# szcompressor/SZ3

Hardware: AMD Instinct MI355X
Metric: compression throughput GB/s + ratio at fixed abs errBound, 512^3 f32 (higher is better)
Workload: dtype f32; 1 GPU; C2: 3D float32 512x512x512 synthetic field per GPU, Lorenzo predictor, abs errBound=0.001, device-resident in -> device-resident Huffman payload; parallelism=slab1, algo=HIP_LORENZO(16), exchange=none (one rank)

## Files before the change

### include/sz3hip.h

```cpp
#ifndef SZ3HIP_H
#define SZ3HIP_H
#include <stddef.h>
#include <stdint.h>
#include "sz3hip_debug.h"

#ifdef __cplusplus
extern "C" {
#endif

#define SZ3HIP_FLOAT 0
#define SZ3HIP_DOUBLE 1
#define SZ3HIP_UINT8 2
#define SZ3HIP_INT8 3
#define SZ3HIP_UINT16 4
#define SZ3HIP_INT16 5
#define SZ3HIP_UINT32 6
#define SZ3HIP_INT32 7
#define SZ3HIP_UINT64 8
#define SZ3HIP_INT64 9

enum { SZ3HIP_EB_ABS = 0, SZ3HIP_EB_REL, SZ3HIP_EB_PSNR, SZ3HIP_EB_L2NORM, SZ3HIP_EB_ABS_AND_REL, SZ3HIP_EB_ABS_OR_REL };

enum {
    SZ3HIP_ALGO_LORENZO_REG = 0,
// ... 136 lines not shown
void sz3hip_set_profiling(sz3hip_ctx *ctx, int on);
int sz3hip_get_stage_times(sz3hip_ctx *ctx, const char **names, float *ms, int max);
void sz3hip_ctx_forget(sz3hip_ctx *ctx);
void sz3hip_ctx_set_speculation(sz3hip_ctx *ctx, int off);
void sz3hip_ctx_set_deterministic(sz3hip_ctx *ctx, int on);
void sz3hip_ctx_set_tuner_exact(sz3hip_ctx *ctx, int on);
void sz3hip_get_spec_stats(const sz3hip_ctx *ctx, uint32_t *hits, uint32_t *misses);
int sz3hip_last_call_fused(const sz3hip_ctx *ctx);
int sz3hip_last_call_q16(const sz3hip_ctx *ctx);
void sz3hip_ctx_set_fused(sz3hip_ctx *ctx, int on);
int sz3hip_lab_build(void);
int sz3hip_debug_copy_codes(sz3hip_ctx *ctx, uint16_t *host_codes, uint64_t n);
int sz3hip_debug_decode_info(sz3hip_ctx *ctx, uint32_t *out4);
void sz3hip_debug_force_generic(int on);
void sz3hip_debug_flags(int flags);

typedef struct sz3hip_comm sz3hip_comm;
#define SZ3HIP_COMM_ID_BYTES 128
sz3hip_comm *sz3hip_comm_create_local(int ndev, const int *devices);
int sz3hip_comm_unique_id(unsigned char *id128);
sz3hip_comm *sz3hip_comm_create_rank(int nranks, int rank, int device, const unsigned char *id128);
void sz3hip_comm_destroy(sz3hip_comm *comm);
int sz3hip_comm_size(const sz3hip_comm *comm);
int sz3hip_comm_rank(const sz3hip_comm *comm);
int sz3hip_comm_local_size(const sz3hip_comm *comm);
int sz3hip_comm_device(const sz3hip_comm *comm, int member);
int sz3hip_comm_allreduce_histogram(sz3hip_comm *comm, sz3hip_ctx *const *ctxs, void *const *streams);
int sz3hip_comm_allreduce_u64(sz3hip_comm *comm, void *const *d_bufs, size_t count, void *const *streams);
int sz3hip_comm_allreduce_minmax(sz3hip_comm *comm, double *mins, double *maxs, void *const *streams);

// ... 11 lines not shown
```

### include/sz3hip_debug.h

```cpp
#ifndef SZ3HIP_DEBUG_H
#define SZ3HIP_DEBUG_H

enum sz3hip_dbg {
    SZ3HIP_DBG_CB_COMPACT_IN_WG = 1,
    SZ3HIP_DBG_K1_LAB_NO_HIST = 1,
    SZ3HIP_DBG_DEC_MULTI_SYM = 2,
    SZ3HIP_DBG_K1_NO_CODE_STORES = 2,
    SZ3HIP_DBG_BLKDEC_FORCE_RETRY = 4,
    SZ3HIP_DBG_K1_V4_NO_STENCIL = 4,
    SZ3HIP_DBG_K1_NO_Q16 = 8,
    SZ3HIP_DBG_BLKDEC_LOCAL_EXPANDED = 16,
    SZ3HIP_DBG_K1_V4_NO_PREFETCH = 16,
    SZ3HIP_DBG_PACK_LAB_NO_STORES = 16,
    SZ3HIP_DBG_K1_NO_MARCH = 32,
    SZ3HIP_DBG_K1_NO_NARROW = 64,
    SZ3HIP_DBG_INTERP_NO_VEC = 128,
    SZ3HIP_DBG_K1_NO_WIDTH_SPEC = 256,
    SZ3HIP_DBG_DEC_NO_FUSED_X = 512,
    SZ3HIP_DBG_PACK_LAB_ONE_UNIT = 512,
    SZ3HIP_DBG_CB_ONE_CLASS = 1024,
    SZ3HIP_DBG_K1_NO_FUSED = 2048,
    SZ3HIP_DBG_BLK_RANK_3_LAUNCHES = 2048,
    SZ3HIP_DBG_BLK_SIDE_8_LAUNCHES = 2048,
    SZ3HIP_DBG_K1_NO_XCD_ORDER = 4096,
// ... 12 lines not shown
    SZ3HIP_DBG_INTERP_LEVELS_ANY_SIZE = 4194304,
    SZ3HIP_DBG_K1_NO_SAMP_IN_LAUNCH = 4194304,
    SZ3HIP_DBG_BLKDEC_BLOCK_PER_WAVE = 8388608,
    SZ3HIP_DBG_K1_Q16_PLAIN_STORES = 8388608,
    SZ3HIP_DBG_K1_NO_DEFER_FOLD = 16777216,
    SZ3HIP_DBG_PACK_NO_SEG_BITS = 33554432,
    SZ3HIP_DBG_BLK_FIT_TILES = 67108864,
    SZ3HIP_DBG_BLK_1D_WAVE_PER_BLOCK = 134217728,
    SZ3HIP_DBG_CTX_NO_PUBLISH_ZERO = 268435456,
    SZ3HIP_DBG_INTERP_HANDOVER_IN_PLACE = 536870912,
    SZ3HIP_DBG_DEC_CARRY_PASS = 536870912,
    SZ3HIP_DBG_BLK_NO_EXIT = 1073741824,
    SZ3HIP_DBG_BLK_NO_SELECT = -2147483647 - 1
};

#endif
```

### sz3_amd/__init__.py

```python
import contextlib
import ctypes as C
import enum
import os

import numpy as np

_HERE = os.path.dirname(os.path.abspath(__file__))
LIB_PATH = os.environ.get("SZ3HIP_LIB") or os.path.join(_HERE, "libsz3hip.so")

EB_ABS, EB_REL, EB_PSNR, EB_L2NORM, EB_ABS_AND_REL, EB_ABS_OR_REL = range(6)
ALGO_LORENZO_REG, ALGO_INTERP_LORENZO, ALGO_INTERP, ALGO_NOPRED, ALGO_LOSSLESS = range(5)
ALGO_HIP_LORENZO = 16
ALGO_HIP_INTERP = 17
INTERP_ALGO_LINEAR, INTERP_ALGO_CUBIC = 0, 1
SZ_FLOAT, SZ_DOUBLE = 0, 1


class Dbg(enum.IntFlag):
    CB_COMPACT_IN_WG = 1
    K1_LAB_NO_HIST = 1
    DEC_MULTI_SYM = 2
    K1_NO_CODE_STORES = 2
    BLKDEC_FORCE_RETRY = 4
    K1_V4_NO_STENCIL = 4
# ... 25 lines not shown
    DEC_DIRECT_STORES = 1048576
    DEC_NO_HALF = 2097152
    INTERP_LEVELS_ANY_SIZE = 4194304
    K1_NO_SAMP_IN_LAUNCH = 4194304
    BLKDEC_BLOCK_PER_WAVE = 8388608
    K1_Q16_PLAIN_STORES = 8388608
    K1_NO_DEFER_FOLD = 16777216
    PACK_NO_SEG_BITS = 33554432
    BLK_FIT_TILES = 67108864
    BLK_1D_WAVE_PER_BLOCK = 134217728
    CTX_NO_PUBLISH_ZERO = 268435456
    INTERP_HANDOVER_IN_PLACE = 536870912
    DEC_CARRY_PASS = 536870912
    BLK_NO_EXIT = 1073741824
    BLK_NO_SELECT = 2147483648


class SZ3HipError(RuntimeError):
    def __init__(self, code, msg):
        super().__init__("sz3hip error %d: %s" % (code, msg))
        self.code = code


class _CConfig(C.Structure):
    _fields_ = [
        ("N", C.c_int32), ("dims", C.c_uint64 * 4), ("num", C.c_uint64),
        ("cmprAlgo", C.c_uint8), ("errorBoundMode", C.c_uint8),
        ("absErrorBound", C.c_double), ("relErrorBound", C.c_double),
        ("psnrErrorBound", C.c_double), ("l2normErrorBound", C.c_double),
        ("openmp", C.c_uint8), ("quantbinCnt", C.c_int32), ("blockSize", C.c_int32),
# ... 234 lines not shown
def _check(rc):
    if rc != 0:
        raise SZ3HipError(rc, lib().sz3hip_last_error().decode())


@contextlib.contextmanager
def debug_flags(flags):
    L = lib()
    L.sz3hip_debug_flags(int(flags))
    try:
        yield
    finally:
        L.sz3hip_debug_flags(0)


_SZ_TYPES = {"float32": 0, "float64": 1, "uint8": 2, "int8": 3, "uint16": 4, "int16": 5, "uint32": 6, "int32": 7, "uint64": 8, "int64": 9}


def _dtype_id(dt):
    dt = np.dtype(dt)
    if dt.name in _SZ_TYPES:
        return _SZ_TYPES[dt.name]
    raise TypeError("sz3_amd supports float32 / float64 and 8 ... 64-bit integers (got %s)" % dt)


class Config:

    _FIELDS = [f[0] for f in _CConfig._fields_ if f[0] not in ("dims",)]

    def __init__(self, *dims):
# ... 544 lines not shown
```

### sz3_amd/csrc/sz3hip_api.cpp

```cpp
#include <hip/hip_runtime.h>

#include <dlfcn.h>
#include <math.h>
#include <stdarg.h>
#include <stdio.h>
#include <stdlib.h>
#include <string.h>

#include <sched.h>
#include <unistd.h>
#include <algorithm>
#include <atomic>
#include <chrono>
#include <mutex>
#include <string>
#include <thread>
#include <vector>

#include "../../include/sz3c.h"
#include "../../include/sz3hip.h"
#include "sz3hip_format.h"
#include "sz3hip_internal.h"
#include "sz3hip_stock_geom.h"
#include "sz3hip_kernels.h"
// ... 1594 lines not shown
        cb.skip_sort = 1;
        int rcb = szk_launch_codebook(ctx->d_hist, &cb, ctx->book_stream);
        if (rcb) return fail(SZ3HIP_EHIP, "codebook kernel launch failed (%d)", rcb);
        HIPCHK(hipEventRecord(ctx->ev_book, ctx->book_stream));
        er.roles = 1;
        er.no_book = 1;
        er.hist = ctx->d_hist;
        er.cb = &cb;
        er.used_lens = ctx->bk[used].lens;
        er.flags = reinterpret_cast<uint32_t *>(ctx->d_counters + 10);
        er.exact = ctx->spec_exact;
    }
    if (how == S2_SAMPLED) {
        er.roles = 1;
        er.no_book = 1;
        er.hist = ctx->d_hist;
        er.cb = &cb;
        er.used_lens = ctx->bk[used].lens;
        er.flags = reinterpret_cast<uint32_t *>(ctx->d_counters + 10);
        er.exact = 1;
    }
    if (how == S2_CLASSIC) {
        if (ctx->range_ready && !cb.range_ready)
            HIPCHK(hipMemsetAsync(ctx->d_counters + 8, 0, 16, s));
        prof_begin(ctx, ST_CODEBOOK, s);
        int rcb = szk_launch_codebook(ctx->d_hist, &cb, s);
        prof_end(ctx, ST_CODEBOOK, s);
        if (rcb) return fail(SZ3HIP_EHIP, "codebook kernel launch failed (%d)", rcb);
    }
    szk_layout_params lp;
// ... 573 lines not shown
    return 1;
#else
    return 0;
#endif
}
extern "C" void sz3hip_ctx_set_fused(sz3hip_ctx *ctx, int on) { ctx->fuse_on = on != 0 && sz3hip_lab_build(); }
extern "C" void sz3hip_get_spec_stats(const sz3hip_ctx *ctx, uint32_t *hits, uint32_t *misses) {
    *hits = ctx->spec_hits;
    *misses = ctx->spec_misses;
}
extern "C" void sz3hip_debug_flags(int flags) {
    szk_dbg_flags = flags;
    szk_interp_novec = (flags & SZ3HIP_DBG_INTERP_NO_VEC) != 0;
    szk_interp_min_blocks = (flags & SZ3HIP_DBG_INTERP_LEVELS_ANY_SIZE) ? 1 : 256;
}
extern "C" int sz3hip_debug_codebook_info(sz3hip_ctx *ctx, uint64_t *out16) {
    HIPCHK(hipSetDevice(ctx->device));
    HIPCHK(hipDeviceSynchronize());
    szk_cb_info info;
    HIPCHK(hipMemcpy(&info, ctx->bk[ctx->book_idx < 0 ? 0 : ctx->book_idx].info, sizeof(info), hipMemcpyDeviceToHost));
    out16[0] = info.n_symbols; out16[1] = info.max_len; out16[2] = info.sym_min; out16[3] = info.sym_count;
    for (int i = 0; i < 12; i++) out16[4 + i] = info.ts[i];
    return 0;
}

extern "C" int sz3hip_debug_decode_info(sz3hip_ctx *ctx, uint32_t *out4) {
    out4[0] = ctx->last_half;
    out4[1] = ctx->last_carry;
    out4[2] = (uint32_t)ctx->half_skip;
    out4[3] = 0;
// ... 287 lines not shown
```

### sz3_amd/csrc/sz3hip_kernels.h

```cpp
#ifndef SZ3HIP_KERNELS_H
#define SZ3HIP_KERNELS_H
#include <hip/hip_runtime.h>
#include <stdint.h>
#include "sz3hip_format.h"
#include "../../include/sz3hip_debug.h"

struct szk_lattice {
    double recip, two_eb, eb;
    float recip_f, two_eb_f, eb_lo_f;
};
static inline szk_lattice szk_make_lattice(double eb) {
    szk_lattice l;
    l.eb = eb;
    l.two_eb = 2.0 * eb;
    l.recip = 1.0 / l.two_eb;
    l.recip_f = (float)l.recip;
    l.two_eb_f = (float)l.two_eb;
    float e = (float)eb;
    if ((double)e > eb) e = __builtin_nextafterf(e, 0.0f);
    l.eb_lo_f = e;
    return l;
}

#define SZK_K1_GRID 2048u
// ... 137 lines not shown
    const uint8_t *side;
    int lists_by_roles;
    int assumed_narrow;
    const uint32_t *q16_flag;
    szk_mode mode;
    const uint32_t *samp_words;
};
struct szk_merge_args {
    const uint32_t *slots;
    const uint32_t *seg_base;
    const uint32_t *fuse_flag;
};
struct szk_encode_roles {
    int roles;
    int no_book;
    const uint64_t *hist;
    const szk_cb_params *cb;
    const uint8_t *used_lens;
    uint32_t *flags;
    int exact;
    const uint32_t *fold_partial;
    uint32_t fold_rows;
    uint64_t *fold_hist;
    uint32_t *fold_range;
};
#define SZK_PACKB_ONLY_SAMPLED 1u
#define SZK_PACKB_LAB_NO_STORES 8u
#define SZK_PACKB_LAB_ONE_UNIT 16u

#define DEC_LUT_BITS 12u
// ... 271 lines not shown
                          uint32_t radius ,
                          uint32_t esc_sym ,
                          uint32_t *zero_word ,
                          const uint16_t *chunk_words, uint64_t n_chunks, uint64_t *group_off, uint64_t *total_words , hipStream_t s);
int szk_launch_decode(const uint8_t *payload, const szk_dec_params *p, uint16_t *codes, uint64_t *chunk_off,
                      uint64_t *total_words, hipStream_t s);
int szk_launch_reconstruct(int x_done, const uint8_t *payload, const szh_header *h, const szh_offsets *o, const uint16_t *codes,
                           void *d_out, void *d_segtot, hipStream_t s, const uint32_t *gate = nullptr,
                           const void *carry = nullptr );
int szk_half_scans_ok(const szh_header *h);
int szk_launch_reconstruct_half(const uint8_t *payload, const szh_header *h, const szh_offsets *o, void *d_half ,
                                void *d_out, uint32_t *ovf, hipStream_t s, const void *carry = nullptr );
void szk_host_offsets(const szh_header *h, szh_offsets *o);
extern int szk_force_generic;
extern int szk_dbg_flags;

#endif
```

### sz3_amd/csrc/sz3hip_kernels.hip

```cpp
#include <hip/hip_runtime.h>
#include <cstddef>
#include <stdint.h>
#include <type_traits>
#include <mutex>
#include <utility>
#include <vector>
#include "sz3hip_format.h"
#include "sz3hip_kernels.h"

#include "sz3hip_devutil.h"

template <typename T>
__global__ __launch_bounds__(256) void k_minmax(const T *__restrict__ in, uint64_t n, double *partial) {
    double mn = INFINITY, mx = -INFINITY;
    bool has_nan = false;
    for (uint64_t i = (uint64_t)blockIdx.x * blockDim.x + threadIdx.x; i < n; i += (uint64_t)gridDim.x * blockDim.x) {
        double v = (double)in[i];
        if (v < mn) mn = v;
        if (v > mx) mx = v;
        has_nan |= (v != v);
    }
    (void)has_nan;
#pragma unroll
    for (int d = WAVE / 2; d > 0; d >>= 1) {
// ... 3498 lines not shown
            tot += s_w[w];
        }
#pragma unroll
        for (int j = 0; j < SCAN_GPT; j++) {
            if (gt + j < n_groups) group_off[gt + j] = run;
            run += sum[j];
        }
        __syncthreads();
        if (threadIdx.x == 0) s_carry += tot;
        __syncthreads();
    }
    if (threadIdx.x == 0) *total_words = s_carry;
}
__global__ __launch_bounds__(256) void k_seg_chunks(const uint16_t *__restrict__ seg_bits, uint64_t n_segs, const uint32_t *seg_made,
                                                    uint16_t *__restrict__ chunk_words, uint64_t n_chunks, uint32_t *__restrict__ group_sums,
                                                    uint16_t *__restrict__ sub_bits) {
    const bool seg_ok = *seg_made != 0;
    const uint64_t n_vec = (n_segs + 7) / 8;
    const uint64_t n_vec16 = (n_vec + 15) / 16 * 16;
    for (uint64_t vi = (uint64_t)blockIdx.x * 256 + threadIdx.x; vi < n_vec16; vi += (uint64_t)gridDim.x * 256) {
        const uint4 q = vi < n_vec ? reinterpret_cast<const uint4 *>(seg_bits)[vi] : make_uint4(0, 0, 0, 0);
        const uint64_t sg0 = vi * 8;
        uint32_t hw[8] = {q.x & 0xFFFF, q.x >> 16, q.y & 0xFFFF, q.y >> 16, q.z & 0xFFFF, q.z >> 16, q.w & 0xFFFF, q.w >> 16};
#pragma unroll
        for (int k = 0; k < 8; k++) hw[k] = (seg_ok && sg0 + k < n_segs) ? hw[k] : 0u;
        const uint32_t cw0 = (hw[0] + hw[1] + hw[2] + hw[3] + 31u) >> 5, cw1 = (hw[4] + hw[5] + hw[6] + hw[7] + 31u) >> 5;
        const uint64_t c = vi * 2;
        if (c + 1 < n_chunks) reinterpret_cast<uint32_t *>(chunk_words)[vi] = cw0 | (cw1 << 16);
        else if (c < n_chunks) chunk_words[c] = (uint16_t)cw0;
        if (sub_bits) {
            constexpr uint32_t SPU = 4 / SZH_SUBS;
// ... 129 lines not shown
    }
#pragma unroll
    for (int k = 0; k < NG; k++) {
        const uint64_t v = gl[k] ? g[k] << (64 - gl[k]) : 0ull;
        const uint32_t word = pos >> 5, sh = pos & 31;
        const uint64_t t = v >> sh;
        const uint32_t w2 = (uint32_t)(((uint64_t)(uint32_t)v << 32) >> sh);
        atomicOr(&stage[word], (uint32_t)(t >> 32));
        atomicOr(&stage[word + 1], (uint32_t)t);
        if (G == 4 || gl[k] + sh > 64) atomicOr(&stage[word + 2], w2);
        pos += gl[k];
    }
    return (total_bits + 31) >> 5;
}

__device__ void assemble_body(const szk_asm_params &p, uint64_t tid, uint64_t nth) {
    __shared__ szh_header s_h0, s_h;
    __shared__ szh_offsets s_o, s_oo;
    if (threadIdx.x == 0) {
        s_h0 = p.state->hdr;
        s_o = p.state->off;
    }
    __syncthreads();
    const szh_header &h0 = s_h0;
    const szh_offsets &o = s_o;
    if (tid == 0) {
        szh_header &h = s_h;
        szh_offsets &oo = s_oo;
        h = s_h0;
        h.bitstream_words = *p.total_words;
        szh_compute_offsets(h, oo);
        h.payload_bytes = oo.end;
        *reinterpret_cast<szh_header *>(p.payload) = h;
        p.state->hdr = h;
        p.state->off = oo;
        p.state->cap_exceeded = oo.end > p.cap;
        for (int i = 0; i < 6; i++) p.state->probe[i] = reinterpret_cast<const uint32_t *>(p.n_vout + 4)[i];
        if (p.assumed_narrow && !szk_is_narrow(p.mode)) atomicOr(&p.state->miss_kind, 32u);
        if (p.q16_flag && *p.q16_flag) atomicOr(&p.state->miss_kind, 128u);
        if (p.samp_words && p.samp_words[SZK_SAMP_READY]) {
            p.state->mispredict = 0;
            p.state->book_miss = 0;
            p.state->n_symbols = 256;
        } else if (!p.lists_by_roles) {
            p.state->mispredict = (uint32_t)p.n_vout[7];
// ... 417 lines not shown
    } else if (!__builtin_amdgcn_ballot_w64(!fit_q)) {
#pragma unroll
        for (int j = 0; j < 4; j++) {
            if (QL[j]) packb_emit(stage, Q[j], QL[j], pos);
            pos += QL[j];
        }
    } else {
#pragma unroll
        for (int k = 0; k < 8; k++) {
            if (PL[k]) packb_emit(stage, P[k], PL[k], pos);
            pos += PL[k];
        }
    }
    return (total_bits + 31u) >> 5;
}
__global__ __launch_bounds__(PB_THREADS) void k_pack_b(const uint16_t *__restrict__ codes, uint64_t n, const uint32_t *__restrict__ g_enc,
                                                        const uint16_t *__restrict__ chunk_words, const uint64_t *__restrict__ group_off, szk_mode mode,
                                                        uint32_t sym_add, const szk_state *__restrict__ state, uint8_t *__restrict__ payload,
                                                        szk_asm_params ap, uint32_t pack_blocks, uint32_t split, szk_role_params rp, uint32_t only_sampled) {
    constexpr int STAGE_WORDS = SZH_CHUNK_SYMS * SZH_MAX_LEN / 32 + 4;
    constexpr uint32_t PB_BATCH = 4;
    constexpr int UNIT_STAGE = PB_BATCH * 128 + 8;
    static_assert(2 * UNIT_STAGE >= STAGE_WORDS && UNIT_STAGE % 2 == 0, "the unit's stage also holds one chunk of the slow tiers");
    __shared__ __align__(16) uint32_t s_pair[128 * 128];
    __shared__ uint32_t s_enc8[256];
    __shared__ uint8_t s_plen8[256];
    __shared__ __align__(16) uint64_t s_stage[PB_WAVES][UNIT_STAGE];
    if ((only_sampled & SZK_PACKB_ONLY_SAMPLED) && !(ap.samp_words && ap.samp_words[SZK_SAMP_READY] && szk_is_narrow(mode))) return;
    const uint32_t roles = rp.on ? ROLE_BLOCKS : 0u;
    if (blockIdx.x < roles) {
        if (threadIdx.x >= 256u) return;
        if (blockIdx.x != 0) role_sort(rp, ap, blockIdx.x == 2, reinterpret_cast<uint8_t *>(s_pair));
        return;
    }
    const uint32_t asm_blocks = gridDim.x - roles - pack_blocks;
    if (blockIdx.x >= roles + pack_blocks) {
        const uint32_t ab = blockIdx.x - roles - pack_blocks;
        assemble_body(ap, (uint64_t)ab * PB_THREADS + threadIdx.x, (uint64_t)asm_blocks * PB_THREADS);
        if (!ap.lists_by_roles) assemble_lists(ap, (uint64_t)ab * PB_THREADS + threadIdx.x, (uint64_t)asm_blocks * PB_THREADS);
        return;
    }
    const uint32_t bid = blockIdx.x - roles;
    if (!szk_is_narrow(mode)) return;
    const uint64_t n_full = n / SZH_CHUNK_SYMS, n_chunks = (n + SZH_CHUNK_SYMS - 1) / SZH_CHUNK_SYMS;
    (void)split;
    const uint32_t wv = (uint32_t)__builtin_amdgcn_readfirstlane((int)(threadIdx.x / WAVE));
    const uint64_t wave_gid = (uint64_t)bid * PB_WAVES + wv, nwaves = (uint64_t)pack_blocks * PB_WAVES;
    const int lane = lane_id();
    const uint8_t *c8 = reinterpret_cast<const uint8_t *>(codes) + (uint64_t)lane * ENC_PER_LANE;
    uint64_t *stage = s_stage[wv];
    uint32_t *out_base = reinterpret_cast<uint32_t *>(payload + state->off.bitstream);
    const uint64_t n_units = (n_full + PB_BATCH - 1) / PB_BATCH;
#ifdef SZ3HIP_LAB
    const bool lab_nost = (only_sampled & SZK_PACKB_LAB_NO_STORES) != 0, lab_nold = (only_sampled & SZK_PACKB_LAB_ONE_UNIT) != 0;
#else
    constexpr bool lab_nost = false, lab_nold = false;
#endif
    struct unit_regs {
        uint4 c[PB_BATCH];
        uint32_t fr;
        uint64_t go;
    };
    auto load_unit = [&](unit_regs &r, uint64_t u) {
        const uint64_t c_lo = u * PB_BATCH, grp = c_lo / PACK_GROUP;
#pragma unroll
        for (uint32_t j = 0; j < PB_BATCH; j++) {
            uint64_t ch = c_lo + j < n_full ? c_lo + j : n_full - 1;
            if (lab_nold) ch %= 4 * nwaves;
            r.c[j] = *reinterpret_cast<const uint4 *>(c8 + ch * SZH_CHUNK_SYMS);
        }
        const uint64_t ci = grp * PACK_GROUP + (uint32_t)lane;
        r.fr = chunk_words[ci < n_chunks ? ci : n_chunks - 1];
        r.go = group_off[grp];
    };
    uint32_t *const stage32 = reinterpret_cast<uint32_t *>(stage);
    uint4 *const stage128 = reinterpret_cast<uint4 *>(stage);
    typedef uint32_t u32x4_dw __attribute__((ext_vector_type(4), aligned(4)));
    auto copy_out = [&](uint32_t *out, uint32_t nw) {
        const uint32_t tail = nw & 3u, w_t = (nw & ~3u) + (uint32_t)lane;
        if ((uint32_t)lane < tail) {
            const uint32_t v = stage32[w_t ^ 1u];
            if (!lab_nost || v == 0x12345678u) out[w_t] = __builtin_bswap32(v);
        }
        __builtin_amdgcn_wave_barrier();
#pragma unroll
        for (uint32_t t = 0; t < PB_BATCH; t++) {
            const uint32_t i = t * WAVE + (uint32_t)lane;
            if (4u * i < nw) {
// ... 12 lines not shown
        __builtin_amdgcn_wave_barrier();
    };
    uint32_t *pend_out = out_base;
    uint32_t pend = 0;
    auto copy_pending = [&]() {
        if (pend) {
            __builtin_amdgcn_fence(__ATOMIC_RELEASE, "workgroup");
            __builtin_amdgcn_wave_barrier();
            copy_out(pend_out, pend);
            pend = 0;
        }
    };
    auto pack_unit = [&](const unit_regs &r, uint64_t unit) {
        const uint64_t c_lo = unit * PB_BATCH;
        const uint32_t first = (uint32_t)(c_lo % PACK_GROUP);
        uint32_t *out = out_base + r.go + wave_sum((uint32_t)lane < first ? r.fr : 0u);
        __builtin_amdgcn_sched_barrier(0);
        copy_pending();
        uint32_t staged = 0;
        auto flush = [&]() {
            if (staged) {
                __builtin_amdgcn_fence(__ATOMIC_RELEASE, "workgroup");
                __builtin_amdgcn_wave_barrier();
                copy_out(out, staged);
                out += staged;
                staged = 0;
            }
        };
#pragma unroll
        for (uint32_t j = 0; j < PB_BATCH; j++) {
            if (c_lo + j < n_full) {
// ... 9 lines not shown
                        stage[i >> 1] = 0;
                        if (lab_nost && v != 0x123456789abcdefull) continue;
                        if (i < nwords) out[i] = __builtin_bswap32((uint32_t)(v >> 32));
                        if (i + 1 < nwords) out[i + 1] = __builtin_bswap32((uint32_t)v);
                    }
                    __builtin_amdgcn_wave_barrier();
                    out += nwords;
                }
            }
        }
        pend_out = out;
        pend = staged;
    };
    uint64_t unit = wave_gid;
    unit_regs ra, rb;
    load_unit(ra, unit < n_units ? unit : n_units - 1);
    if (threadIdx.x < 256u) {
        const uint32_t e = g_enc[threadIdx.x != 255u ? threadIdx.x + sym_add : 0u];
        s_enc8[threadIdx.x] = e >> 5;
        s_plen8[threadIdx.x] = (uint8_t)(e & 31u);
    }
    for (int i = lane; i < UNIT_STAGE; i += WAVE) stage[i] = 0;
    __syncthreads();
    for (uint32_t i = threadIdx.x; i < 128u * 128u; i += PB_THREADS) {
        const uint32_t i1 = i >> 7, i0 = (i & 127u) ^ i1;
        const uint32_t t0 = i0 < 64u ? i0 + 128u : i0, t1 = i1 < 64u ? i1 + 128u : i1;
        const uint32_t l0 = s_plen8[t0], l1 = s_plen8[t1];
        const uint32_t len = l0 + l1;
        s_pair[i] = (l0 && l1 && len <= 27u) ? ((((s_enc8[t0] << l1) | s_enc8[t1]) << 5) | len) : 0u;
    }
    __syncthreads();
    while (unit < n_units) {
        uint64_t nu = unit + nwaves;
        load_unit(rb, nu < n_units ? nu : unit);
        __builtin_amdgcn_sched_barrier(0);
        pack_unit(ra, unit);
        unit = nu;
        if (unit >= n_units) break;
        nu = unit + nwaves;
        load_unit(ra, nu < n_units ? nu : unit);
        __builtin_amdgcn_sched_barrier(0);
        pack_unit(rb, unit);
        unit = nu;
    }
    copy_pending();
    if (n_full < n_chunks && wave_gid == 0) {
// ... 14 lines not shown
        const uint32_t incl = wave_incl_scan(bits);
        const uint32_t total_bits = (uint32_t)__builtin_amdgcn_readlane((int)incl, WAVE - 1);
        uint32_t pos = incl - bits;
#pragma unroll
        for (int k = 0; k < 8; k++) {
            if (PL[k]) packb_emit(stage, P[k], PL[k], pos);
            pos += PL[k];
        }
        const uint32_t nwords = (total_bits + 31u) >> 5;
        const uint64_t grp = n_full / PACK_GROUP;
        const uint32_t cin = (uint32_t)(n_full % PACK_GROUP);
        uint32_t bp = (uint32_t)lane < cin ? chunk_words[grp * PACK_GROUP + lane] : 0u;
        const uint32_t before = wave_sum(bp);
        __builtin_amdgcn_fence(__ATOMIC_RELEASE, "workgroup");
        __builtin_amdgcn_wave_barrier();
        uint32_t *out = out_base + group_off[grp] + before;
        for (uint32_t i = lane; i < nwords; i += WAVE) out[i] = __builtin_bswap32((uint32_t)(stage[i >> 1] >> ((i & 1u) ? 0 : 32)));
    }
}

#ifdef SZ3HIP_LAB
struct szk_merge_params {
    const uint32_t *slots;
    const uint16_t *seg_bits;
    const uint32_t *seg_base;
    const uint32_t *fuse_flag;
};
#define MERGE_BLOCK 16
__global__ __launch_bounds__(256) void k_merge(szk_merge_params mp, uint64_t n, const uint16_t *__restrict__ chunk_words,
                                               const uint64_t *__restrict__ group_off, szk_mode mode, const szk_state *__restrict__ state,
                                               uint8_t *__restrict__ payload, szk_asm_params ap, uint32_t pack_blocks, szk_role_params rp) {
// ... 1254 lines not shown
    SZK_CHECK_LAUNCH();
    return 0;
}

int szk_launch_minmax(int dtype, const void *d_in, uint64_t n, double *d_partial, double *d_out, hipStream_t s) {
    const int nb = 1024;
    if (dtype == 0) hipLaunchKernelGGL(k_minmax<float>, dim3(nb), dim3(256), 0, s, (const float *)d_in, n, d_partial);
    else hipLaunchKernelGGL(k_minmax<double>, dim3(nb), dim3(256), 0, s, (const double *)d_in, n, d_partial);
    hipLaunchKernelGGL(k_minmax_final, dim3(1), dim3(64), 0, s, d_partial, nb, d_out);
    SZK_CHECK_LAUNCH();
    return 0;
}

int szk_force_generic = 0;
int szk_dbg_flags = 0;

static uint32_t k1_grid(const void *kernel, uint64_t ntiles) {
    static int n_cu = 0;
    if (!n_cu) {
        int dev = 0;
        hipDeviceProp_t prop;
        if (hipGetDevice(&dev) == hipSuccess && hipGetDeviceProperties(&prop, dev) == hipSuccess) n_cu = prop.multiProcessorCount;
        if (n_cu <= 0) n_cu = 256;
    }
    static std::mutex occ_mu;
    static std::vector<std::pair<const void *, int>> occ;
    int per_cu = 0;
    {
        std::lock_guard<std::mutex> lk(occ_mu);
        for (const auto &e : occ)
// ... 258 lines not shown
    const uint64_t n_chunks = (n + SZH_CHUNK_SYMS - 1) / SZH_CHUNK_SYMS;
    const uint64_t nb = (n_chunks + 3) / 4;
    if (nb > 0x7FFFFFFFull) return -1;
    const uint32_t sym_add = (uint32_t)radius - 127u;
    const uint32_t pgrid = (uint32_t)(nb < 2048 ? nb : 2048);
    uint16_t *sub_bits = asmp ? asmp->sub_bits : nullptr;
    if (!seg_bits) hipLaunchKernelGGL(k_chunk_bits2, dim3(pgrid), dim3(256), 0, s, codes, n, d_enc, info, mode, sym_add, chunk_words, sub_bits);
    szk_fold_params fp{};
    if (er && er->fold_rows) {
        fp.partial = er->fold_partial;
        fp.nrows = er->fold_rows;
        fp.win_lo = radius - HIST_WIN / 2;
        fp.hist = er->fold_hist;
        fp.range = er->fold_range;
    }
    const uint16_t *scan_in = nullptr;
    if (seg_bits) {
        const uint64_t n_segs = (n + 255) / 256;
        uint32_t *gsums = reinterpret_cast<uint32_t *>(group_off + (n_chunks + PACK_GROUP - 1) / PACK_GROUP + 1);
        hipLaunchKernelGGL(k_seg_chunks, dim3((uint32_t)std::min<uint64_t>(((n_segs + 7) / 8 + 255) / 256, 1024)), dim3(256), 0, s, seg_bits, n_segs, seg_made,
                           chunk_words, n_chunks, gsums, sub_bits);
        scan_in = reinterpret_cast<const uint16_t *>(gsums);
    }
    hipLaunchKernelGGL(k_scan_groups, dim3(fp.nrows ? 65 : 1), dim3(1024), 0, s, chunk_words, n_chunks, group_off, total_words, *layout, 1, scan_in,
                       (uint64_t)0, seg_made, fp);
    szk_role_params rp{};
    szk_asm_params apv = asmp ? *asmp : szk_asm_params{};
    if (er && er->roles && asmp) {
        rp.on = 1;
        rp.no_book = er->no_book ? 1u : 0u;
        rp.hist = er->hist;
        rp.cb = *er->cb;
        rp.used = info;
        rp.used_lens = er->used_lens;
        rp.flags = er->flags;
        rp.need_seg = seg_bits != nullptr;
        rp.exact = er->exact;
        apv.lists_by_roles = 1;
    }
    const uint32_t rb = rp.on ? ROLE_BLOCKS : 0u;
    const uint32_t extra = rb + (asmp ? 32u : 0u);
    constexpr uint32_t ASM_BLOCKS = 32;
#ifdef SZ3HIP_LAB
    if (mg) {
        szk_merge_params mp;
        mp.slots = mg->slots;
        mp.seg_bits = seg_bits;
        mp.seg_base = mg->seg_base;
        mp.fuse_flag = mg->fuse_flag;
        const uint32_t pb = pgrid < 2048 - extra ? pgrid : 2048 - extra;
        hipLaunchKernelGGL(k_merge, dim3(rb + pb + (asmp ? ASM_BLOCKS : 0)), dim3(256), 0, s, mp, n, chunk_words, group_off, mode, state, payload, apv, pb, rp);
    } else
#else
    if (mg) return -2;
#endif
    if (asmp && !(rp.on && !rp.no_book) && n_chunks >= 4096 && ((asmp->assumed_narrow && !(szk_dbg_flags & SZ3HIP_DBG_PACK_OLD)) || asmp->samp_words)) {
        static int n_cu = 0;
        if (!n_cu) {
            int dev = 0;
            hipDeviceProp_t prop;
            if (hipGetDevice(&dev) == hipSuccess && hipGetDeviceProperties(&prop, dev) == hipSuccess) n_cu = prop.multiProcessorCount;
            if (n_cu <= 0) n_cu = 256;
        }
        const uint32_t pb = (uint32_t)n_cu > rb + 1 ? (uint32_t)n_cu - rb : 1u;
        const uint32_t split = 1;
        uint32_t beside = asmp->samp_words && !asmp->assumed_narrow ? SZK_PACKB_ONLY_SAMPLED : 0u;
#ifdef SZ3HIP_LAB
        beside |= (szk_dbg_flags & SZ3HIP_DBG_PACK_LAB_NO_STORES) ? SZK_PACKB_LAB_NO_STORES : 0u;
        beside |= (szk_dbg_flags & SZ3HIP_DBG_PACK_LAB_ONE_UNIT) ? SZK_PACKB_LAB_ONE_UNIT : 0u;
#endif
        hipLaunchKernelGGL(k_pack_b, dim3(rb + PB_ASM_BLOCKS + pb), dim3(PB_THREADS), 0, s, codes, n, d_enc, chunk_words, group_off, mode, sym_add, state,
                           payload, apv, pb, split, rp, beside);
        if (beside & SZK_PACKB_ONLY_SAMPLED) {
            const uint32_t pb2 = pgrid < 1280 - extra ? pgrid : 1280 - extra;
            hipLaunchKernelGGL((k_pack<ENC_WIN>), dim3(rb + pb2 + (asmp ? ASM_BLOCKS : 0)), dim3(256), 0, s, codes, n, d_enc, info, chunk_words, group_off, mode,
                               sym_add, state, payload, apv, pb2, rp);
        }
    } else if (mode.pack_wide) {
        const uint32_t pb = pgrid < 768 - extra ? pgrid : 768 - extra;
        hipLaunchKernelGGL((k_pack<2 * ENC_WIN>), dim3(rb + pb + (asmp ? ASM_BLOCKS : 0)), dim3(256), 0, s, codes, n, d_enc, info, chunk_words, group_off, mode,
                           sym_add, state, payload, apv, pb, rp);
    } else {
        const uint32_t pb = pgrid < 1280 - extra ? pgrid : 1280 - extra;
        hipLaunchKernelGGL((k_pack<ENC_WIN>), dim3(rb + pb + (asmp ? ASM_BLOCKS : 0)), dim3(256), 0, s, codes, n, d_enc, info, chunk_words, group_off, mode,
                           sym_add, state, payload, apv, pb, rp);
    }
    SZK_CHECK_LAUNCH();
    return 0;
}
__global__ __launch_bounds__(256) void k_publish(const szk_state *__restrict__ state, uint32_t *host_state, uint32_t *host_seq, uint32_t seq,
                                                 uint4 *zero, uint32_t zero_vec16, const uint64_t *blk_others, uint4 *zero_blk0, uint4 *zero_blk1) {
    if (blockIdx.x == 0) {
        const uint32_t *src = reinterpret_cast<const uint32_t *>(state);
        constexpr uint32_t OW = offsetof(szk_state, blk_others) / 4;
        for (uint32_t i = threadIdx.x; i < sizeof(szk_state) / 4; i += 256) {
            uint32_t v = src[i];
            if (blk_others && (i == OW || i == OW + 1)) v = reinterpret_cast<const uint32_t *>(blk_others)[i - OW];
            __hip_atomic_store(&host_state[i], v, __ATOMIC_RELAXED, __HIP_MEMORY_SCOPE_SYSTEM);
        }
        __threadfence_system();
// ... 249 lines not shown
```

Baseline: 2349 GB/s.

## Fuse group-offset scan into pack_b kernel, dropping k_scan_groups launch

```diff
diff --git a/include/sz3hip.h b/include/sz3hip.h
--- a/include/sz3hip.h
+++ b/include/sz3hip.h
@@ -174,6 +174,8 @@
 int sz3hip_debug_decode_info(sz3hip_ctx *ctx, uint32_t *out4);
 void sz3hip_debug_force_generic(int on);
 void sz3hip_debug_flags(int flags);
+void sz3hip_debug_flags2(int flags);
+int sz3hip_last_encode_launches(void);
 
 typedef struct sz3hip_comm sz3hip_comm;
 #define SZ3HIP_COMM_ID_BYTES 128
diff --git a/include/sz3hip_debug.h b/include/sz3hip_debug.h
--- a/include/sz3hip_debug.h
+++ b/include/sz3hip_debug.h
@@ -50,4 +50,8 @@
     SZ3HIP_DBG_BLK_NO_SELECT = -2147483647 - 1
 };
 
+enum sz3hip_dbg2 {
+    SZ3HIP_DBG2_PACK_SCAN_LAUNCH = 1
+};
+
 #endif
diff --git a/sz3_amd/__init__.py b/sz3_amd/__init__.py
--- a/sz3_amd/__init__.py
+++ b/sz3_amd/__init__.py
@@ -63,6 +63,10 @@
     DEC_CARRY_PASS = 536870912
     BLK_NO_EXIT = 1073741824
     BLK_NO_SELECT = 2147483648
+
+
+class Dbg2(enum.IntFlag):
+    PACK_SCAN_LAUNCH = 1
 
 
 class SZ3HipError(RuntimeError):
@@ -327,6 +331,20 @@
         L.sz3hip_debug_flags(0)
 
 
+@contextlib.contextmanager
+def debug_flags2(flags):
+    L = lib()
+    L.sz3hip_debug_flags2(int(flags))
+    try:
+        yield
+    finally:
+        L.sz3hip_debug_flags2(0)
+
+
+def last_encode_launches():
+    return int(lib().sz3hip_last_encode_launches())
+
+
 _SZ_TYPES = {"float32": 0, "float64": 1, "uint8": 2, "int8": 3, "uint16": 4, "int16": 5, "uint32": 6, "int32": 7, "uint64": 8, "int64": 9}
 
 
diff --git a/sz3_amd/csrc/sz3hip_api.cpp b/sz3_amd/csrc/sz3hip_api.cpp
--- a/sz3_amd/csrc/sz3hip_api.cpp
+++ b/sz3_amd/csrc/sz3hip_api.cpp
@@ -1632,6 +1632,7 @@
     if (how == S2_SAMPLED) {
         er.roles = 1;
         er.no_book = 1;
+        er.sampled = 1;
         er.hist = ctx->d_hist;
         er.cb = &cb;
         er.used_lens = ctx->bk[used].lens;
@@ -2235,6 +2236,8 @@
     szk_interp_novec = (flags & SZ3HIP_DBG_INTERP_NO_VEC) != 0;
     szk_interp_min_blocks = (flags & SZ3HIP_DBG_INTERP_LEVELS_ANY_SIZE) ? 1 : 256;
 }
+extern "C" void sz3hip_debug_flags2(int flags) { szk_dbg_flags2 = flags; }
+extern "C" int sz3hip_last_encode_launches(void) { return szk_encode_launches; }
 extern "C" int sz3hip_debug_codebook_info(sz3hip_ctx *ctx, uint64_t *out16) {
     HIPCHK(hipSetDevice(ctx->device));
     HIPCHK(hipDeviceSynchronize());
diff --git a/sz3_amd/csrc/sz3hip_kernels.h b/sz3_amd/csrc/sz3hip_kernels.h
--- a/sz3_amd/csrc/sz3hip_kernels.h
+++ b/sz3_amd/csrc/sz3hip_kernels.h
@@ -175,6 +175,7 @@
 struct szk_encode_roles {
     int roles;
     int no_book;
+    int sampled;
     const uint64_t *hist;
     const szk_cb_params *cb;
     const uint8_t *used_lens;
@@ -476,5 +477,7 @@
 void szk_host_offsets(const szh_header *h, szh_offsets *o);
 extern int szk_force_generic;
 extern int szk_dbg_flags;
+extern int szk_dbg_flags2;
+extern int szk_encode_launches;
 
 #endif
diff --git a/sz3_amd/csrc/sz3hip_kernels.hip b/sz3_amd/csrc/sz3hip_kernels.hip
--- a/sz3_amd/csrc/sz3hip_kernels.hip
+++ b/sz3_amd/csrc/sz3hip_kernels.hip
@@ -3536,7 +3536,8 @@
 }
 __global__ __launch_bounds__(256) void k_seg_chunks(const uint16_t *__restrict__ seg_bits, uint64_t n_segs, const uint32_t *seg_made,
                                                     uint16_t *__restrict__ chunk_words, uint64_t n_chunks, uint32_t *__restrict__ group_sums,
-                                                    uint16_t *__restrict__ sub_bits) {
+                                                    uint16_t *__restrict__ sub_bits, szk_layout_params lp, int do_layout) {
+    if (do_layout && blockIdx.x == 0 && threadIdx.x == 255) layout_pre(lp);
     const bool seg_ok = *seg_made != 0;
     const uint64_t n_vec = (n_segs + 7) / 8;
     const uint64_t n_vec16 = (n_vec + 15) / 16 * 16;
@@ -3696,7 +3697,7 @@
     return (total_bits + 31) >> 5;
 }
 
-__device__ void assemble_body(const szk_asm_params &p, uint64_t tid, uint64_t nth) {
+__device__ void assemble_body(const szk_asm_params &p, uint64_t tid, uint64_t nth, const uint64_t *total_in = nullptr) {
     __shared__ szh_header s_h0, s_h;
     __shared__ szh_offsets s_o, s_oo;
     if (threadIdx.x == 0) {
@@ -3710,7 +3711,7 @@
         szh_header &h = s_h;
         szh_offsets &oo = s_oo;
         h = s_h0;
-        h.bitstream_words = *p.total_words;
+        h.bitstream_words = total_in ? *total_in : *p.total_words;
         szh_compute_offsets(h, oo);
         h.payload_bytes = oo.end;
         *reinterpret_cast<szh_header *>(p.payload) = h;
@@ -4158,10 +4159,14 @@
     }
     return (total_bits + 31u) >> 5;
 }
+#define PB_SCAN_GROUPS 4096u
+template <bool SCAN>
 __global__ __launch_bounds__(PB_THREADS) void k_pack_b(const uint16_t *__restrict__ codes, uint64_t n, const uint32_t *__restrict__ g_enc,
                                                         const uint16_t *__restrict__ chunk_words, const uint64_t *__restrict__ group_off, szk_mode mode,
                                                         uint32_t sym_add, const szk_state *__restrict__ state, uint8_t *__restrict__ payload,
-                                                        szk_asm_params ap, uint32_t pack_blocks, uint32_t split, szk_role_params rp, uint32_t only_sampled) {
+                                                        szk_asm_params ap, uint32_t pack_blocks, uint32_t split, szk_role_params rp, uint32_t only_sampled,
+                                                        const uint32_t *__restrict__ group_sums, uint32_t n_groups, uint64_t *__restrict__ group_off_w,
+                                                        uint64_t *__restrict__ total_w) {
     constexpr int STAGE_WORDS = SZH_CHUNK_SYMS * SZH_MAX_LEN / 32 + 4;
     constexpr uint32_t PB_BATCH = 4;
     constexpr int UNIT_STAGE = PB_BATCH * 128 + 8;
@@ -4170,6 +4175,18 @@
     __shared__ uint32_t s_enc8[256];
     __shared__ uint8_t s_plen8[256];
     __shared__ __align__(16) uint64_t s_stage[PB_WAVES][UNIT_STAGE];
+    __shared__ __align__(16) uint32_t s_goff[SCAN ? PB_SCAN_GROUPS : 4u];
+    __shared__ uint32_t s_gw[PB_WAVES];
+    __shared__ uint64_t s_total;
+    auto load_sums = [&]() -> uint4 {
+        const uint32_t g0 = 4u * threadIdx.x;
+        uint4 q = make_uint4(0u, 0u, 0u, 0u);
+        if (g0 < n_groups) q = *reinterpret_cast<const uint4 *>(group_sums + g0);
+        q.y = g0 + 1u < n_groups ? q.y : 0u;
+        q.z = g0 + 2u < n_groups ? q.z : 0u;
+        q.w = g0 + 3u < n_groups ? q.w : 0u;
+        return q;
+    };
     if ((only_sampled & SZK_PACKB_ONLY_SAMPLED) && !(ap.samp_words && ap.samp_words[SZK_SAMP_READY] && szk_is_narrow(mode))) return;
     const uint32_t roles = rp.on ? ROLE_BLOCKS : 0u;
     if (blockIdx.x < roles) {
@@ -4180,7 +4197,18 @@
     const uint32_t asm_blocks = gridDim.x - roles - pack_blocks;
     if (blockIdx.x >= roles + pack_blocks) {
         const uint32_t ab = blockIdx.x - roles - pack_blocks;
-        assemble_body(ap, (uint64_t)ab * PB_THREADS + threadIdx.x, (uint64_t)asm_blocks * PB_THREADS);
+        if (SCAN && ab == 0) {
+            const uint4 q = load_sums();
+            const uint32_t ws = wave_sum(q.x + q.y + q.z + q.w);
+            if (lane_id() == 0) s_gw[threadIdx.x / WAVE] = ws;
+            __syncthreads();
+            if (threadIdx.x == 0) {
+                uint64_t t = 0;
+                for (uint32_t w = 0; w < PB_WAVES; w++) t += s_gw[w];
+                s_total = t;
+            }
+        }
+        assemble_body(ap, (uint64_t)ab * PB_THREADS + threadIdx.x, (uint64_t)asm_blocks * PB_THREADS, SCAN ? &s_total : nullptr);
         if (!ap.lists_by_roles) assemble_lists(ap, (uint64_t)ab * PB_THREADS + threadIdx.x, (uint64_t)asm_blocks * PB_THREADS);
         return;
     }
@@ -4205,7 +4233,7 @@
         uint32_t fr;
         uint64_t go;
     };
-    auto load_unit = [&](unit_regs &r, uint64_t u) {
+    auto load_unit_mem = [&](unit_regs &r, uint64_t u) {
         const uint64_t c_lo = u * PB_BATCH, grp = c_lo / PACK_GROUP;
 #pragma unroll
         for (uint32_t j = 0; j < PB_BATCH; j++) {
@@ -4215,7 +4243,11 @@
         }
         const uint64_t ci = grp * PACK_GROUP + (uint32_t)lane;
         r.fr = chunk_words[ci < n_chunks ? ci : n_chunks - 1];
-        r.go = group_off[grp];
+        if (!SCAN) r.go = group_off[grp];
+    };
+    auto load_unit = [&](unit_regs &r, uint64_t u) {
+        load_unit_mem(r, u);
+        if (SCAN) r.go = s_goff[(u * PB_BATCH) / PACK_GROUP];
     };
     uint32_t *const stage32 = reinterpret_cast<uint32_t *>(stage);
     uint4 *const stage128 = reinterpret_cast<uint4 *>(stage);
@@ -4258,7 +4290,8 @@
     auto pack_unit = [&](const unit_regs &r, uint64_t unit) {
         const uint64_t c_lo = unit * PB_BATCH;
         const uint32_t first = (uint32_t)(c_lo % PACK_GROUP);
-        uint32_t *out = out_base + r.go + wave_sum((uint32_t)lane < first ? r.fr : 0u);
+        const uint64_t go = SCAN ? (uint64_t)(uint32_t)__builtin_amdgcn_readfirstlane((int)(uint32_t)r.go) : r.go;
+        uint32_t *out = out_base + go + wave_sum((uint32_t)lane < first ? r.fr : 0u);
         __builtin_amdgcn_sched_barrier(0);
         copy_pending();
         uint32_t staged = 0;
@@ -4298,7 +4331,15 @@
     };
     uint64_t unit = wave_gid;
     unit_regs ra, rb;
-    load_unit(ra, unit < n_units ? unit : n_units - 1);
+    uint4 gq = make_uint4(0u, 0u, 0u, 0u);
+    uint32_t g_mine = 0, g_incl = 0;
+    if (SCAN) gq = load_sums();
+    load_unit_mem(ra, unit < n_units ? unit : n_units - 1);
+    if (SCAN) {
+        g_mine = gq.x + gq.y + gq.z + gq.w;
+        g_incl = wave_incl_scan(g_mine);
+        if (lane == WAVE - 1) s_gw[wv] = g_incl;
+    }
     if (threadIdx.x < 256u) {
         const uint32_t e = g_enc[threadIdx.x != 255u ? threadIdx.x + sym_add : 0u];
         s_enc8[threadIdx.x] = e >> 5;
@@ -4306,6 +4347,19 @@
     }
     for (int i = lane; i < UNIT_STAGE; i += WAVE) stage[i] = 0;
     __syncthreads();
+    if (SCAN) {
+        uint32_t run = g_incl - g_mine;
+        for (uint32_t w = 0; w < PB_WAVES; w++) run += w < wv ? s_gw[w] : 0u;
+        const uint4 o = make_uint4(run, run + gq.x, run + gq.x + gq.y, run + gq.x + gq.y + gq.z);
+        reinterpret_cast<uint4 *>(s_goff)[threadIdx.x] = o;
+        if (bid == 0) {
+            const uint32_t g0 = 4u * threadIdx.x, ov[4] = {o.x, o.y, o.z, o.w};
+#pragma unroll
+            for (uint32_t k = 0; k < 4; k++)
+                if (g0 + k < n_groups) group_off_w[g0 + k] = ov[k];
+            if (threadIdx.x == PB_THREADS - 1u) *total_w = (uint64_t)run + g_mine;
+        }
+    }
     for (uint32_t i = threadIdx.x; i < 128u * 128u; i += PB_THREADS) {
         const uint32_t i1 = i >> 7, i0 = (i & 127u) ^ i1;
         const uint32_t t0 = i0 < 64u ? i0 + 128u : i0, t1 = i1 < 64u ? i1 + 128u : i1;
@@ -4314,6 +4368,7 @@
         s_pair[i] = (l0 && l1 && len <= 27u) ? ((((s_enc8[t0] << l1) | s_enc8[t1]) << 5) | len) : 0u;
     }
     __syncthreads();
+    if (SCAN) ra.go = s_goff[((unit < n_units ? unit : n_units - 1) * PB_BATCH) / PACK_GROUP];
     while (unit < n_units) {
         uint64_t nu = unit + nwaves;
         load_unit(rb, nu < n_units ? nu : unit);
@@ -4358,7 +4413,7 @@
         const uint32_t before = wave_sum(bp);
         __builtin_amdgcn_fence(__ATOMIC_RELEASE, "workgroup");
         __builtin_amdgcn_wave_barrier();
-        uint32_t *out = out_base + group_off[grp] + before;
+        uint32_t *out = out_base + (SCAN ? (uint64_t)s_goff[grp] : group_off[grp]) + before;
         for (uint32_t i = lane; i < nwords; i += WAVE) out[i] = __builtin_bswap32((uint32_t)(stage[i >> 1] >> ((i & 1u) ? 0 : 32)));
     }
 }
@@ -5643,6 +5698,8 @@
 
 int szk_force_generic = 0;
 int szk_dbg_flags = 0;
+int szk_dbg_flags2 = 0;
+int szk_encode_launches = 0;
 
 static uint32_t k1_grid(const void *kernel, uint64_t ntiles) {
     static int n_cu = 0;
@@ -5931,16 +5988,6 @@
         fp.hist = er->fold_hist;
         fp.range = er->fold_range;
     }
-    const uint16_t *scan_in = nullptr;
-    if (seg_bits) {
-        const uint64_t n_segs = (n + 255) / 256;
-        uint32_t *gsums = reinterpret_cast<uint32_t *>(group_off + (n_chunks + PACK_GROUP - 1) / PACK_GROUP + 1);
-        hipLaunchKernelGGL(k_seg_chunks, dim3((uint32_t)std::min<uint64_t>(((n_segs + 7) / 8 + 255) / 256, 1024)), dim3(256), 0, s, seg_bits, n_segs, seg_made,
-                           chunk_words, n_chunks, gsums, sub_bits);
-        scan_in = reinterpret_cast<const uint16_t *>(gsums);
-    }
-    hipLaunchKernelGGL(k_scan_groups, dim3(fp.nrows ? 65 : 1), dim3(1024), 0, s, chunk_words, n_chunks, group_off, total_words, *layout, 1, scan_in,
-                       (uint64_t)0, seg_made, fp);
     szk_role_params rp{};
     szk_asm_params apv = asmp ? *asmp : szk_asm_params{};
     if (er && er->roles && asmp) {
@@ -5956,6 +6003,27 @@
         apv.lists_by_roles = 1;
     }
     const uint32_t rb = rp.on ? ROLE_BLOCKS : 0u;
+    const bool packb = !mg && asmp && !(rp.on && !rp.no_book) && n_chunks >= 4096 &&
+                       ((asmp->assumed_narrow && !(szk_dbg_flags & SZ3HIP_DBG_PACK_OLD)) || asmp->samp_words);
+    uint32_t beside = packb && asmp->samp_words && !asmp->assumed_narrow ? SZK_PACKB_ONLY_SAMPLED : 0u;
+    const uint64_t n_groups = (n_chunks + PACK_GROUP - 1) / PACK_GROUP;
+    const bool scan_in_pack = packb && seg_bits && er && er->sampled && !beside && n_groups <= PB_SCAN_GROUPS && !fp.nrows &&
+                              !(szk_dbg_flags2 & SZ3HIP_DBG2_PACK_SCAN_LAUNCH);
+    uint32_t *gsums = reinterpret_cast<uint32_t *>(group_off + ((n_groups + 2) & ~1ull));
+    const uint16_t *scan_in = nullptr;
+    szk_encode_launches = 0;
+    if (seg_bits) {
+        const uint64_t n_segs = (n + 255) / 256;
+        hipLaunchKernelGGL(k_seg_chunks, dim3((uint32_t)std::min<uint64_t>(((n_segs + 7) / 8 + 255) / 256, 1024)), dim3(256), 0, s, seg_bits, n_segs, seg_made,
+                           chunk_words, n_chunks, gsums, sub_bits, *layout, scan_in_pack ? 1 : 0);
+        scan_in = reinterpret_cast<const uint16_t *>(gsums);
+    }
+    szk_encode_launches++;
+    if (!scan_in_pack) {
+        hipLaunchKernelGGL(k_scan_groups, dim3(fp.nrows ? 65 : 1), dim3(1024), 0, s, chunk_words, n_chunks, group_off, total_words, *layout, 1, scan_in,
+                           (uint64_t)0, seg_made, fp);
+        szk_encode_launches++;
+    }
     const uint32_t extra = rb + (asmp ? 32u : 0u);
     constexpr uint32_t ASM_BLOCKS = 32;
 #ifdef SZ3HIP_LAB
@@ -5967,11 +6035,12 @@
         mp.fuse_flag = mg->fuse_flag;
         const uint32_t pb = pgrid < 2048 - extra ? pgrid : 2048 - extra;
         hipLaunchKernelGGL(k_merge, dim3(rb + pb + (asmp ? ASM_BLOCKS : 0)), dim3(256), 0, s, mp, n, chunk_words, group_off, mode, state, payload, apv, pb, rp);
+        szk_encode_launches++;
     } else
 #else
     if (mg) return -2;
 #endif
-    if (asmp && !(rp.on && !rp.no_book) && n_chunks >= 4096 && ((asmp->assumed_narrow && !(szk_dbg_flags & SZ3HIP_DBG_PACK_OLD)) || asmp->samp_words)) {
+    if (packb) {
         static int n_cu = 0;
         if (!n_cu) {
             int dev = 0;
@@ -5981,26 +6050,33 @@
         }
         const uint32_t pb = (uint32_t)n_cu > rb + 1 ? (uint32_t)n_cu - rb : 1u;
         const uint32_t split = 1;
-        uint32_t beside = asmp->samp_words && !asmp->assumed_narrow ? SZK_PACKB_ONLY_SAMPLED : 0u;
 #ifdef SZ3HIP_LAB
         beside |= (szk_dbg_flags & SZ3HIP_DBG_PACK_LAB_NO_STORES) ? SZK_PACKB_LAB_NO_STORES : 0u;
         beside |= (szk_dbg_flags & SZ3HIP_DBG_PACK_LAB_ONE_UNIT) ? SZK_PACKB_LAB_ONE_UNIT : 0u;
 #endif
-        hipLaunchKernelGGL(k_pack_b, dim3(rb + PB_ASM_BLOCKS + pb), dim3(PB_THREADS), 0, s, codes, n, d_enc, chunk_words, group_off, mode, sym_add, state,
-                           payload, apv, pb, split, rp, beside);
+        if (scan_in_pack)
+            hipLaunchKernelGGL(k_pack_b<true>, dim3(rb + PB_ASM_BLOCKS + pb), dim3(PB_THREADS), 0, s, codes, n, d_enc, chunk_words, (const uint64_t *)nullptr, mode,
+                               sym_add, state, payload, apv, pb, split, rp, beside, (const uint32_t *)gsums, (uint32_t)n_groups, group_off, total_words);
+        else
+            hipLaunchKernelGGL(k_pack_b<false>, dim3(rb + PB_ASM_BLOCKS + pb), dim3(PB_THREADS), 0, s, codes, n, d_enc, chunk_words, group_off, mode, sym_add,
+                               state, payload, apv, pb, split, rp, beside, (const uint32_t *)nullptr, 0u, (uint64_t *)nullptr, (uint64_t *)nullptr);
+        szk_encode_launches++;
         if (beside & SZK_PACKB_ONLY_SAMPLED) {
             const uint32_t pb2 = pgrid < 1280 - extra ? pgrid : 1280 - extra;
             hipLaunchKernelGGL((k_pack<ENC_WIN>), dim3(rb + pb2 + (asmp ? ASM_BLOCKS : 0)), dim3(256), 0, s, codes, n, d_enc, info, chunk_words, group_off, mode,
                                sym_add, state, payload, apv, pb2, rp);
+            szk_encode_launches++;
         }
     } else if (mode.pack_wide) {
         const uint32_t pb = pgrid < 768 - extra ? pgrid : 768 - extra;
         hipLaunchKernelGGL((k_pack<2 * ENC_WIN>), dim3(rb + pb + (asmp ? ASM_BLOCKS : 0)), dim3(256), 0, s, codes, n, d_enc, info, chunk_words, group_off, mode,
                            sym_add, state, payload, apv, pb, rp);
+        szk_encode_launches++;
     } else {
         const uint32_t pb = pgrid < 1280 - extra ? pgrid : 1280 - extra;
         hipLaunchKernelGGL((k_pack<ENC_WIN>), dim3(rb + pb + (asmp ? ASM_BLOCKS : 0)), dim3(256), 0, s, codes, n, d_enc, info, chunk_words, group_off, mode,
                            sym_add, state, payload, apv, pb, rp);
+        szk_encode_launches++;
     }
     SZK_CHECK_LAUNCH();
     return 0;
```

Result: faster. 2383 GB/s (median of 6 runs) (+1.4%).
